# keurfonluu/stochopy

Hardware: AMD Instinct MI355X
Metric: objective-fn evals/sec (higher is better)
Workload: dtype f64

## Files before the change

include/stochopy_hip.h:

```cpp
#ifndef STOCHOPY_HIP_H
#define STOCHOPY_HIP_H

#include <stdint.h>

#ifdef __cplusplus
extern "C" {
#endif

#define SX_ABI_VERSION 1

enum {
    SX_FUN_ACKLEY = 0,
    SX_FUN_GRIEWANK = 1,
    SX_FUN_QUARTIC = 2,
    SX_FUN_RASTRIGIN = 3,
    SX_FUN_ROSENBROCK = 4,
    SX_FUN_SPHERE = 5,
    SX_FUN_STYBLINSKI_TANG = 6,
    SX_FUN_COUNT = 7
};

enum { SX_DE_RAND1BIN = 0, SX_DE_RAND2BIN = 1, SX_DE_BEST1BIN = 2, SX_DE_BEST2BIN = 3 };

enum {
// ... 4 lines not shown
#define SX_STATUS_NONE 100

int sx_abi_version(void);
const char *sx_last_error(void);
int sx_device_count(void);
int sx_struct_size(int which);

int sx_sum_plan(int64_t m, int32_t *out, int cap);
int64_t sx_fun_terms(int fun_id, int n);

int64_t sx_num_partials(int64_t P, int n);
int sx_rows_per_workgroup(int n);
int sx_wide_from(void);
int64_t sx_de_num_partials(int64_t P, int n, int wide_from);
int sx_eval(int fun_id, const double *X, int64_t P, int n, int64_t ldx, const double *xm, const double *xstd,
            double *f, double *part_f, int64_t *part_i, void *stream);

int sx_philox_lhs(double *X, int64_t rows, int n, int64_t ld, int64_t row0, int64_t P, const double *lower,
                  const double *upper, uint32_t key0, uint32_t key1, void *stream);

int sx_argmin(const double *f, int64_t P, double *ws_f, int64_t *ws_i, int64_t ws_len, int64_t *out_idx,
              double *out_val, void *stream);

typedef struct sx_state {
    int64_t it;
    int64_t gbidx;
    double gfit;
    double dx;
    int32_t status;
    int32_t done;
    int64_t reserved[3];
} sx_state;

typedef struct sx_de_args {
    double *buf0, *buf1;
    double *fit;
    double *candfit;
    double *gbest;
    const double *lower;
    const double *upper;
    sx_state *state;
    double *part_f;
    int64_t *part_i;
    const double *r1;
    const int32_t *donors;
    const int32_t *irand;
    const double *resample;
    int64_t P;
    int64_t ld;
    int64_t row0;
    int32_t n;
    int32_t fun_id;
    int32_t strategy;
    int32_t constraints;
    int32_t rng;
    int32_t maxiter;
    int32_t wide_from;
    int32_t pad;
    double F, CR, xtol, ftol;
    uint32_t key0, key1;
} sx_de_args;

int sx_de_generation(const sx_de_args *a, int finalize, void *stream);

int sx_select_finalize(const double *part_f, const int64_t *part_i, int64_t npart, const double *rows0,
                       const double *rows1, int64_t ld, int n, double *gbest, sx_state *state, int maxiter,
                       double xtol, double ftol, void *stream);

int sx_shard_best(const double *part_f, const int64_t *part_i, int64_t npart, const double *rows0,
                  const double *rows1, int64_t ld, int n, const sx_state *state, int64_t row0, double *record,
                  void *stream);
int sx_gather_finalize(const double *records, int world, int n, double *gbest, sx_state *state, int maxiter,
                       double xtol, double ftol, void *stream);
int sx_de_shard_generation(const struct sx_de_args *a, double *record, void *stream);

typedef struct sx_graph sx_graph;
int sx_de_graph_create(const sx_de_args *a, int ngen, sx_graph **out);
int sx_de_chain_launch(const sx_de_args *a, int parity, int finalize_only, void *stream);
int sx_de_chain_graph_create(const sx_de_args *a, int ngen, int start_parity, sx_graph **out);
int sx_graph_launch(sx_graph *g, void *stream);
int sx_graph_destroy(sx_graph *g);

#define SX_MAX_PEERS 8
#define SX_IPC_HANDLE_BYTES 64
typedef struct sx_xchg_args {
    uint64_t *peer[SX_MAX_PEERS];
    int32_t world, rank;
    int64_t timeout_ticks;
    int32_t *error;
    uint64_t *relay;
    const double *pop0[SX_MAX_PEERS];
    const double *pop1[SX_MAX_PEERS];
// ... 204 lines not shown
```

stochopy_amd/_lib.py:

```python
import ctypes as C
import os

_HERE = os.path.dirname(os.path.abspath(__file__))
LIB_PATH = os.path.join(_HERE, "lib", "libstochopy_hip.so")

SX_STATUS_NONE = 100
NARROW_DIM, WIDE_DIM = 4096, 262144


def wide_from():
    return int(lib().sx_wide_from())
SX_RNG_HOST, SX_RNG_PHILOX = 0, 1

FUN_IDS = {
    "ackley": 0,
    "griewank": 1,
    "quartic": 2,
    "rastrigin": 3,
    "rosenbrock": 4,
    "sphere": 5,
    "styblinski_tang": 6,
}
DE_STRATEGIES = {"rand1bin": 0, "rand2bin": 1, "best1bin": 2, "best2bin": 3}
DE_DONORS = {"rand1bin": 3, "rand2bin": 5, "best1bin": 2, "best2bin": 4}

vp = C.c_void_p
i64 = C.c_int64
i32 = C.c_int32
f64 = C.c_double


class SxState(C.Structure):
    _fields_ = [("it", i64), ("gbidx", i64), ("gfit", f64), ("dx", f64), ("status", i32), ("done", i32),
                ("reserved", i64 * 3)]


class SxDeArgs(C.Structure):
    _fields_ = [
        ("buf0", vp), ("buf1", vp), ("fit", vp), ("candfit", vp), ("gbest", vp), ("lower", vp),
        ("upper", vp), ("state", vp), ("part_f", vp), ("part_i", vp), ("r1", vp), ("donors", vp),
        ("irand", vp), ("resample", vp),
        ("P", i64), ("ld", i64), ("row0", i64),
        ("n", i32), ("fun_id", i32), ("strategy", i32), ("constraints", i32), ("rng", i32), ("maxiter", i32),
        ("wide_from", i32), ("pad", i32),
        ("F", f64), ("CR", f64), ("xtol", f64), ("ftol", f64),
        ("key0", C.c_uint32), ("key1", C.c_uint32),
    ]


class SxPsoArgs(C.Structure):
    _fields_ = [
        ("X", vp), ("V", vp), ("pbest", vp), ("pbestfit", vp), ("candfit", vp), ("gbest", vp), ("lower", vp),
        ("upper", vp), ("state", vp), ("part_f", vp), ("part_i", vp), ("r1", vp), ("r2", vp), ("pending_restart", vp),
        ("P", i64), ("ld", i64), ("row0", i64),
        ("n", i32), ("fun_id", i32), ("constraints", i32), ("rng", i32), ("maxiter", i32), ("pad", i32),
        ("w", f64), ("c1", f64), ("c2", f64), ("xtol", f64), ("ftol", f64),
        ("key0", C.c_uint32), ("key1", C.c_uint32),
    ]


SX_MAX_PEERS = 8
SX_IPC_HANDLE_BYTES = 64


class SxXchgArgs(C.Structure):
    _fields_ = [("peer", vp * SX_MAX_PEERS), ("world", i32), ("rank", i32), ("timeout_ticks", i64), ("error", vp),
                ("relay", vp), ("pop0", vp * SX_MAX_PEERS), ("pop1", vp * SX_MAX_PEERS), ("global_rows", i64),
                ("shard_rows", i64)]


class SxCmaState(C.Structure):
    _fields_ = [("it", i64), ("nfev", i64), ("best_row", i64), ("fbest", f64), ("sigma", f64), ("sigma_next", f64),
                ("tmp_coef", f64), ("psnorm", f64), ("status", i32), ("done", i32), ("stop_it", i64),
                ("reserved", f64 * 6)]


class SxVdArgs(C.Structure):
    _fields_ = [
# ... 159 lines not shown
```

stochopy_amd/csrc/sx_async.hip:

```cpp
#ifndef SX_ASYNC_PART
#define SX_ASYNC_PART 0
#endif
#define SX_FUSED_TAIL_BY_LANE 0
#include "sx_device.hpp"
#include "sx_host.hpp"
#include "sx_rowops.hpp"

namespace sx {
int make_plan_arg(int fun_id, int n, PlanArg *out);
}
using namespace sx;

namespace {

#ifndef SX_SWEEP_WAVES
#define SX_SWEEP_WAVES 16
#endif
constexpr int kSweepWaves = SX_SWEEP_WAVES;
__host__ __device__ constexpr int sweep_waves(int fun_id) {
    return (fun_id == SX_FUN_ACKLEY || fun_id == SX_FUN_GRIEWANK) ? (kSweepWaves + 1) / 2 : kSweepWaves;
}
constexpr int kSweepSlots = 64;

struct SweepGeometry {
// ... 335 lines not shown
template <int RNG, int LPR, int NFIX = 0>
pso_async_t pick_pso(int fun_id) {
    switch (fun_id) {
        case SX_FUN_ACKLEY: return pso_async_kernel<SX_FUN_ACKLEY, RNG, LPR, NFIX>;
        case SX_FUN_RASTRIGIN: return pso_async_kernel<SX_FUN_RASTRIGIN, RNG, LPR, NFIX>;
        case SX_FUN_ROSENBROCK: return pso_async_kernel<SX_FUN_ROSENBROCK, RNG, LPR, NFIX>;
        case SX_FUN_SPHERE: return pso_async_kernel<SX_FUN_SPHERE, RNG, LPR, NFIX>;
        case SX_FUN_GRIEWANK: return pso_async_kernel<SX_FUN_GRIEWANK, RNG, LPR, 0>;
        case SX_FUN_QUARTIC: return pso_async_kernel<SX_FUN_QUARTIC, RNG, LPR, 0>;
        case SX_FUN_STYBLINSKI_TANG: return pso_async_kernel<SX_FUN_STYBLINSKI_TANG, RNG, LPR, 0>;
    }
    return nullptr;
}

template <typename K>
int launch_sweep(K kern, const SweepGeometry &g, hipStream_t s, const void *args_struct) {
    (void)args_struct;
    SX_HIP(hipFuncSetAttribute(reinterpret_cast<const void *>(kern), hipFuncAttributeMaxDynamicSharedMemorySize,
                               (int)g.lds));
    return 0;
}

}

#if SX_ASYNC_PART == 0
extern "C" int sx_de_async_generation(const sx_de_args *a, void *stream) {
    SX_REQUIRE(a != nullptr, "sx_de_async: null args");
    SX_REQUIRE(a->buf0 && a->fit && a->gbest && a->state, "sx_de_async: null device pointer");
    SX_REQUIRE(a->P >= 2 && a->P < (int64_t)1 << 31 && a->n >= 1 && a->n <= kMaxDim && a->ld >= a->n, "sx_de_async: bad shape");
    SX_REQUIRE(a->fun_id >= 0 && a->fun_id < SX_FUN_COUNT, "sx_de_async: unknown objective");
    SX_REQUIRE(a->strategy >= 0 && a->strategy <= SX_DE_BEST2BIN, "sx_de_async: unknown strategy");
    SX_REQUIRE(a->P - 1 >= donors_of(a->strategy), "sx_de_async: population too small for the strategy");
    SX_REQUIRE(a->rng == SX_RNG_HOST || a->rng == SX_RNG_PHILOX, "sx_de_async: unknown rng mode");
    SX_REQUIRE(a->rng != SX_RNG_HOST || (a->r1 && a->donors && a->irand), "sx_de_async: host draws missing");
    SX_REQUIRE(a->constraints == 0 || (a->lower && a->upper && (a->rng != SX_RNG_HOST || a->resample)),
               "sx_de_async: bounds / resample draws missing");
    PlanArg plan;
    if (make_plan_arg(a->fun_id, a->n, &plan)) return -1;
    de_async_t kern = nullptr;
    if (a->rng == SX_RNG_PHILOX) {
        SX_DISPATCH_LPR(a->n, kern = a->n == 4 * LPR ? (pick_de<SX_RNG_PHILOX, LPR, 4 * LPR>(a->fun_id))
                                                      : (pick_de<SX_RNG_PHILOX, LPR>(a->fun_id)))
    } else {
        SX_DISPATCH_LPR(a->n, kern = (pick_de<SX_RNG_HOST, LPR>(a->fun_id)))
    }
    const SweepGeometry g = sweep_geometry(a->n, 0, a->fun_id);
    if (int rc = launch_sweep(kern, g, (hipStream_t)stream, a)) return rc;
    hipLaunchKernelGGL(kern, dim3(1), dim3(g.waves * kWave), g.lds, (hipStream_t)stream, *a, plan);
    SX_LAUNCH_CHECK();
    return 0;
}

#else
extern "C" int sx_pso_async_generation(const sx_pso_args *a, void *stream) {
    SX_REQUIRE(a != nullptr, "sx_pso_async: null args");
    SX_REQUIRE(a->X && a->V && a->pbest && a->pbestfit && a->gbest && a->state, "sx_pso_async: null device pointer");
    SX_REQUIRE(a->P >= 2 && a->n >= 1 && a->n <= kMaxDim && a->ld >= a->n, "sx_pso_async: bad shape");
    SX_REQUIRE(a->fun_id >= 0 && a->fun_id < SX_FUN_COUNT, "sx_pso_async: unknown objective");
    SX_REQUIRE(a->rng == SX_RNG_HOST || a->rng == SX_RNG_PHILOX, "sx_pso_async: unknown rng mode");
    SX_REQUIRE(a->rng != SX_RNG_HOST || (a->r1 && a->r2), "sx_pso_async: host draws missing");
    SX_REQUIRE(a->constraints == 0 || (a->lower && a->upper), "sx_pso_async: bounds missing");
    PlanArg plan;
    if (make_plan_arg(a->fun_id, a->n, &plan)) return -1;
    pso_async_t kern = nullptr;
    if (a->rng == SX_RNG_PHILOX) {
        SX_DISPATCH_LPR(a->n, kern = a->n == 4 * LPR ? (pick_pso<SX_RNG_PHILOX, LPR, 4 * LPR>(a->fun_id))
// ... 12 lines not shown
```

stochopy_amd/csrc/sx_de.hip:

```cpp
#define SX_DE_XM 0
#include "sx_de_kernel.hpp"
#include "sx_wide.hpp"

namespace sx {
void *de_chain_kernel(int fun_id, int n, int64_t P, int strategy, int constraints);
void *de_p2p_kernel(int fun_id, int n, int64_t P, int strategy, int constraints);
}

namespace {

int check_args(const sx_de_args *a) {
    SX_REQUIRE(a != nullptr, "sx_de: null args");
    SX_REQUIRE(a->buf0 && a->buf1 && a->fit && a->state && a->part_f && a->part_i, "sx_de: null device pointer");
    SX_REQUIRE(a->P >= 2 && a->P < (int64_t)1 << 31 && a->n >= 1 && a->ld >= a->n, "sx_de: bad shape");
    SX_REQUIRE(a->fun_id >= 0 && a->fun_id < SX_FUN_COUNT, "sx_de: unknown objective");
    SX_REQUIRE(a->strategy >= 0 && a->strategy <= 3, "sx_de: unknown strategy");
    SX_REQUIRE(a->P - 1 >= donors_of(a->strategy), "sx_de: popsize too small for the strategy");
    SX_REQUIRE(a->rng == SX_RNG_HOST || a->rng == SX_RNG_PHILOX, "sx_de: unknown rng mode");
    if (a->rng == SX_RNG_HOST) {
        SX_REQUIRE(a->r1 && a->donors && a->irand, "sx_de: host draws missing");
        SX_REQUIRE(a->constraints == 0 || a->resample, "sx_de: resample block missing");
    }
    SX_REQUIRE(a->constraints == 0 || (a->lower && a->upper), "sx_de: bounds missing");
    return 0;
}

de_kernel_t kernel_for(const sx_de_args *a) {
    return a->rng == SX_RNG_PHILOX ? pick_kernel<SX_RNG_PHILOX, 0>(a->fun_id, a->n, a->P, a->strategy, a->constraints)
                                   : pick_kernel<SX_RNG_HOST, 0>(a->fun_id, a->n, a->P, a->strategy, a->constraints);
}

Geometry geometry(const sx_de_args *a) {
    Geometry g = row_geometry(a->P, a->n, de_wide_from(a));
    if (!is_wide(a->n, de_wide_from(a))) g.lds = (size_t)rows_per_block(a->n) * gen_row_stride(a->n) * sizeof(double);
    return g;
}

}

extern "C" int sx_de_generation(const sx_de_args *a, int finalize, void *stream) {
    if (int rc = check_args(a)) return rc;
    hipStream_t s = (hipStream_t)stream;
    const Geometry g = geometry(a);
    if (is_wide(a->n, de_wide_from(a))) {
        if (int rc = wide_de_launch(a, s)) return rc;
    } else {
        PlanArg plan;
        if (make_plan_arg(a->fun_id, a->n, &plan)) return -1;
        hipLaunchKernelGGL(kernel_for(a), dim3(g.blocks), dim3(g.threads), g.lds, s, (const sx_state *)nullptr,
                           (const double *)nullptr, (const int64_t *)nullptr, (int64_t)g.blocks, *a, plan, 0, 0,
                           sx_xchg_args{});
        SX_LAUNCH_CHECK();
    }
    if (finalize) {
        SX_REQUIRE(a->gbest != nullptr, "sx_de_generation: the separate finalize kernel needs the gbest buffer");
        return sx_select_finalize(a->part_f, a->part_i, g.blocks, a->buf0, a->buf1, a->ld, a->n, a->gbest, a->state,
                                  a->maxiter, a->xtol, a->ftol, stream);
    }
    return 0;
}

extern "C" int sx_de_graph_create(const sx_de_args *a, int ngen, sx_graph **out) {
    if (int rc = check_args(a)) return rc;
    SX_REQUIRE(out != nullptr && ngen >= 1 && a->gbest != nullptr, "sx_de_graph_create: bad arguments");
    SX_REQUIRE(a->rng == SX_RNG_PHILOX, "sx_de_graph_create: graphs need in-kernel (Philox) draws");
    PlanArg plan = {};
    const bool wide = is_wide(a->n, de_wide_from(a));
    if (!wide && make_plan_arg(a->fun_id, a->n, &plan)) return -1;
    const Geometry g = geometry(a);
    sx_graph *gr = new sx_graph();
    SX_HIP(hipGraphCreate(&gr->graph, 0));
    sx_de_args args = *a;
    int zero = 0;
    int64_t npart = g.blocks;
    sx_xchg_args nox = {};
    const void *none = nullptr;
    void *kargs[] = {&none, &none, &none, &npart, &args, &plan, &zero, &zero, &nox};
    hipGraphNode_t prev = nullptr;
    for (int i = 0; i < ngen; ++i) {
        if (wide) {
            if (int rc = wide_de_add_node(gr->graph, &prev, a)) return rc;
        } else {
            hipKernelNodeParams kp = {};
            kp.func = (void *)kernel_for(a);
            kp.gridDim = dim3(g.blocks);
            kp.blockDim = dim3(g.threads);
            kp.sharedMemBytes = (unsigned)g.lds;
            kp.kernelParams = kargs;
            kp.extra = nullptr;
            hipGraphNode_t node;
            SX_HIP(hipGraphAddKernelNode(&node, gr->graph, prev ? &prev : nullptr, prev ? 1 : 0, &kp));
            prev = node;
        }
        if (int rc = add_finalize_node(gr->graph, &prev, a->part_f, a->part_i, g.blocks, a->buf0, a->buf1, a->ld, a->n,
                                       a->gbest, a->state, a->maxiter, a->xtol, a->ftol))
            return rc;
    }
    SX_HIP(hipGraphInstantiate(&gr->exec, gr->graph, nullptr, nullptr, 0));
    *out = gr;
    return 0;
}

extern "C" int sx_de_shard_generation(const sx_de_args *a, double *record, void *stream) {
    SX_REQUIRE(record != nullptr, "sx_de_shard_generation: null record");
    if (int rc = sx_de_generation(a, 0, stream)) return rc;
    return sx_shard_best(a->part_f, a->part_i, (int64_t)geometry(a).blocks, a->buf0, a->buf1, a->ld, a->n, a->state,
                         a->row0, record, stream);
}

static int check_chain(const sx_de_args *a, bool peer_exchange) {
    if (int rc = check_args(a)) return rc;
    SX_REQUIRE(a->rng == SX_RNG_PHILOX, "sx_de_chain: needs in-kernel (Philox) draws");
    SX_REQUIRE(!is_wide(a->n, de_wide_from(a)), "sx_de_chain: rows served by the one-workgroup-per-row kernels (n > wide_from) take the two-kernel path (sx_de_generation)");
    SX_REQUIRE(peer_exchange || geometry(a).blocks <= 512,
               "sx_de_chain: more than 512 workgroup records (use the two-kernel path)");
    return 0;
}

static int chain_launch(const sx_de_args *a, const sx_xchg_args *x, int parity, int finalize_only, void *stream) {
    if (int rc = check_chain(a, x != nullptr)) return rc;
    SX_REQUIRE(parity == 0 || parity == 1, "sx_de_chain_launch: parity must be 0 or 1");
    PlanArg plan;
    if (make_plan_arg(a->fun_id, a->n, &plan)) return -1;
    const Geometry g = geometry(a);
    de_kernel_t kern = (de_kernel_t)(x ? de_p2p_kernel(a->fun_id, a->n, a->P, a->strategy, a->constraints)
                                       : de_chain_kernel(a->fun_id, a->n, a->P, a->strategy, a->constraints));
    const unsigned blocks = finalize_only ? 1u : g.blocks + (x ? 1u : 0u);
    hipLaunchKernelGGL(kern, dim3(blocks), dim3(g.threads), g.lds, (hipStream_t)stream,
                       (const sx_state *)(a->state + parity), (const double *)(a->part_f + (int64_t)parity * g.blocks),
                       (const int64_t *)(a->part_i + (int64_t)parity * g.blocks), (int64_t)g.blocks, *a, plan, parity,
                       finalize_only ? 1 : 0, x ? *x : sx_xchg_args{});
    SX_LAUNCH_CHECK();
    return 0;
}

static int chain_graph_create(const sx_de_args *a, const sx_xchg_args *x, int ngen, int start_parity, sx_graph **out) {
    if (int rc = check_chain(a, x != nullptr)) return rc;
    SX_REQUIRE(out != nullptr && ngen >= 1 && (start_parity == 0 || start_parity == 1),
               "sx_de_chain_graph_create: bad arguments");
    PlanArg plan;
    if (make_plan_arg(a->fun_id, a->n, &plan)) return -1;
    const Geometry g = geometry(a);
    sx_graph *gr = new sx_graph();
    SX_HIP(hipGraphCreate(&gr->graph, 0));
    sx_de_args args = *a;
    sx_xchg_args xa = x ? *x : sx_xchg_args{};
    int mode = 0;
    int64_t npart = g.blocks;
    hipGraphNode_t prev = nullptr;
    for (int i = 0; i < ngen; ++i) {
        int parity = (start_parity + i) & 1;
        const sx_state *sin_pre = a->state + parity;
        const double *pf_pre = a->part_f + (int64_t)parity * npart;
        const int64_t *pi_pre = a->part_i + (int64_t)parity * npart;
        void *kargs[] = {&sin_pre, &pf_pre, &pi_pre, &npart, &args, &plan, &parity, &mode, &xa};
        hipKernelNodeParams kp = {};
        kp.func = x ? de_p2p_kernel(a->fun_id, a->n, a->P, a->strategy, a->constraints)
                    : de_chain_kernel(a->fun_id, a->n, a->P, a->strategy, a->constraints);
        kp.gridDim = dim3(g.blocks + (x ? 1u : 0u));
        kp.blockDim = dim3(g.threads);
        kp.sharedMemBytes = (unsigned)g.lds;
        kp.kernelParams = kargs;
        kp.extra = nullptr;
        hipGraphNode_t node;
        SX_HIP(hipGraphAddKernelNode(&node, gr->graph, prev ? &prev : nullptr, prev ? 1 : 0, &kp));
        prev = node;
    }
    SX_HIP(hipGraphInstantiate(&gr->exec, gr->graph, nullptr, nullptr, 0));
    *out = gr;
    return 0;
}

extern "C" int sx_de_chain_launch(const sx_de_args *a, int parity, int finalize_only, void *stream) {
    return chain_launch(a, nullptr, parity, finalize_only, stream);
}
extern "C" int sx_de_chain_graph_create(const sx_de_args *a, int ngen, int start_parity, sx_graph **out) {
    return chain_graph_create(a, nullptr, ngen, start_parity, out);
}

extern "C" int sx_de_p2p_launch(const sx_de_args *a, const sx_xchg_args *x, int parity, int finalize_only,
                                void *stream) {
    if (int rc = check_xchg_args(x)) return rc;
    return chain_launch(a, x, parity, finalize_only, stream);
}
extern "C" int sx_de_p2p_graph_create(const sx_de_args *a, const sx_xchg_args *x, int ngen, int start_parity,
                                      sx_graph **out) {
    if (int rc = check_xchg_args(x)) return rc;
    return chain_graph_create(a, x, ngen, start_parity, out);
// ... 17 lines not shown
```

stochopy_amd/csrc/sx_de_kernel.hpp:

```cpp
#pragma once
#ifndef SX_DE_XM
#error "define SX_DE_XM (0, 1 or 2) before including sx_de_kernel.hpp"
#endif
#include <type_traits>
#include <vector>

#include "sx_device.hpp"
#include "sx_host.hpp"
#include "sx_rowops.hpp"
#include "sx_xchg.hpp"

namespace sx {
int make_plan_arg(int fun_id, int n, PlanArg *out);
int add_finalize_node(hipGraph_t graph, hipGraphNode_t *prev, const double *part_f, const int64_t *part_i,
                      int64_t npart, const double *rows0, const double *rows1, int64_t ld, int n, double *gbest,
                      sx_state *state, int maxiter, double xtol, double ftol);
int check_xchg_args(const sx_xchg_args *x);
}
using namespace sx;

#if defined(SX_TRACE) && SX_DE_XM == 1
__device__ unsigned long long sx_trace_buf[1024 * 16];
#define SX_TP(k)                                                                              \
    do {                                                                                      \
// ... 117 lines not shown
        int status = SX_STATUS_NONE;
        if (it >= 2) {
            if (gf <= a.ftol)
                status = 1;
            else if (it >= a.maxiter)
                status = -1;
        }
        sx_state *so = a.state + (mode == 1 ? 2 : 1 - chain_p);
        so->it = it;
        so->gbidx = gi;
        so->gfit = gf;
        so->dx = 0.0;
        so->status = status;
        so->done = status != SX_STATUS_NONE;
        so->reserved[0] = prev_winner;
        so->reserved[1] = winner;
    }
}

constexpr int kStep = 4;

#ifndef SX_DE_NFIX_WAVES
#define SX_DE_NFIX_WAVES 1
#endif
#ifndef SX_DE_WAVE_ROWS_WAVES
#define SX_DE_WAVE_ROWS_WAVES 1
#endif
template <int FUN, int RNG, int XM, int LPR, bool FULL, int NFIX = 0, int STRAT = -1, bool ONEB = false>
__global__ __launch_bounds__(kMaxWavesPerBlock *kWave, (NFIX != 0 && XM <= 1) ? SX_DE_NFIX_WAVES
                                                       : (NFIX == 0 && XM == 0 && STRAT >= 0 && LPR == kWave) ? SX_DE_WAVE_ROWS_WAVES
                                                                                                                 : 1) void de_generation_kernel(const sx_state *const sin_pre,
                                                                                 const double *const pf_pre,
                                                                                 const int64_t *const pi_pre,
                                                                                 const int64_t npart,
                                                                                 const sx_de_args a,
                                                                                 const PlanArg plan,
                                                                                 const int chain_p, const int mode,
                                                                                 const sx_xchg_args x) {
    constexpr bool CHAIN = XM >= 1;
    constexpr bool P2P = XM == 2;
    extern __shared__ __attribute__((aligned(16))) double lds[];
    __shared__ double sf[kMaxRowsPerBlock];
    __shared__ int64_t si[kMaxRowsPerBlock];
    __shared__ double s_gf;
    __shared__ int64_t s_gi;
    __shared__ int s_winner;
    SX_TP(0);
    const int n = NFIX ? NFIX : a.n;
    const int64_t P = a.P, ld = a.ld;
    const RowIds<LPR> id(P, P2P ? 1 : 0);
    const int l = id.l;
    const int64_t rowc = id.rowc;
    double *U = lds + id.slot * gen_row_stride(n);

    const sx_state *sin = (CHAIN && !P2P) ? sin_pre : CHAIN ? a.state + chain_p : a.state;
    constexpr int kRecPerLane = 8;
    double pfv[kRecPerLane];
    using rec_t = typename std::conditional<LPR == kWave, int32_t, int64_t>::type;
    constexpr rec_t kNoRec = LPR == kWave ? (rec_t)INT32_MAX : (rec_t)INT64_MAX;
    rec_t piv[kRecPerLane];
#ifndef SX_CHAIN_REC_WAVE0
#define SX_CHAIN_REC_WAVE0 1
#endif
    if (CHAIN && !P2P && (!SX_CHAIN_REC_WAVE0 || id.wave == 0)) {
        const double *pf = pf_pre;
        const int64_t *pi = pi_pre;
        const int per = (int)((npart + kWave - 1) / kWave);
        const int64_t k0 = (int64_t)id.lane * per;
#pragma unroll
        for (int u = 0; u < kRecPerLane; ++u) {
            const bool in = u < per && k0 + u < npart;
            pfv[u] = in ? pf[k0 + u] : __builtin_huge_val();
            piv[u] = in ? (rec_t)pi[k0 + u] : kNoRec;
        }
    }
    if (P2P && blockIdx.x == 0) {
        p2p_service(a, x, chain_p, mode, npart, sin, LPR == kWave);
        return;
    }
    if (sin->done) {
        if (CHAIN && mode == 1 && threadIdx.x == 0) a.state[2] = *sin;
        return;
    }
    const int64_t it = CHAIN ? sin->it + 1 : sin->it;
    SX_TP(6);

    const uint32_t gen = (uint32_t)(it + 1);
    const double *__restrict__ cur = (it & 1) ? a.buf1 : a.buf0;
    double *__restrict__ nxt = (it & 1) ? a.buf0 : a.buf1;
    const double fold = a.fit[rowc];
    const double *__restrict__ xi = cur + rowc * ld;
    const uint32_t grow = (uint32_t)(a.row0 + rowc);
    const int strategy = STRAT >= 0 ? STRAT : a.strategy;
    const int k = donors_of(strategy);
    const bool repair = STRAT >= 0 ? false : a.constraints != 0;
    const bool use_best = strategy == SX_DE_BEST1BIN || strategy == SX_DE_BEST2BIN;

    int64_t d[kMaxDonors];
    int irand;
    const bool gdon = P2P && x.global_rows > 0;
    if (RNG == SX_RNG_PHILOX) {
        philox_donors(gdon ? x.global_rows : P, k, gdon ? a.row0 + rowc : rowc, grow, gen, a.key0, a.key1, n, d, irand);
    } else {
#pragma unroll
        for (int t = 0; t < kMaxDonors; ++t) d[t] = t < k ? (int64_t)a.donors[(int64_t)t * P + rowc] : 0;
        irand = a.irand[rowc];
    }
    SX_TP(1);
// ... 229 lines not shown
            for (int t = 0; t < kStep; ++t) {
                const int e = (q0 + t) * LPR + l;
                g[t] = (use_best && (FULL || e < n)) ? gb[e] : 0.0;
            }
        }
#pragma unroll
        for (int t = 0; t < kStep; ++t) {
            const int e = (q0 + t) * LPR + l;
            if (FULL || e < n) {
                const double v = de_mutant(strategy, g[t], bd[0][t], bd[1][t], bd[2][t], bd[3][t], bd[4][t], F);
                double cand = (e == irand || br[t] <= CR) ? v : bx[t];
                if (repair && (cand < a.lower[e] || cand > a.upper[e])) cand = brs[t];
                U[e] = cand;
                if (kRegRow) keep[t] = cand;
            }
        }
    };
    if constexpr (LPR < kWave) {
        trial_batch(0, B0);
    } else {
        trial_batch(0, B0);
        if constexpr (!ONEB) {
            for (int q0 = kStep; q0 < nq; q0 += kStep) {
                load_batch(q0, B0);
                trial_batch(q0, B0);
            }
        }
    }

    SX_TP(2);
    const double fc = row_objective<FUN, LPR, FULL, NFIX, SX_LONG_STATIC, ONEB>(U, n, plan, l);
    SX_TP(3);
    const bool better = fc < fold;
    if (FULL || id.active) {
        double *__restrict__ xo = nxt + id.row * ld;
        if constexpr (kRegRow) {
#pragma unroll
            for (int t = 0; t < kStep; ++t)
                if (NFIX != 0 || l + t * LPR < n) st_stream(xo + l + t * LPR, better ? keep[t] : B0.x[t]);
        } else {
            const double *__restrict__ src = better ? U : xi;
            for (int e0 = l; e0 < n; e0 += kStep * LPR) {
                double v[kStep];
#pragma unroll
                for (int t = 0; t < kStep; ++t) v[t] = (FULL || e0 + t * LPR < n) ? src[e0 + t * LPR] : 0.0;
#pragma unroll
                for (int t = 0; t < kStep; ++t)
                    if (FULL || e0 + t * LPR < n) xo[e0 + t * LPR] = v[t];
            }
        }
        if (l == 0) {
            if (better) a.fit[id.row] = fc;
            if (a.candfit != nullptr) a.candfit[id.row] = fc;
        }
    }
    SX_TP(4);
    block_partial<LPR>(better ? fc : fold, id, sf, si, part_f_out, part_i_out);
    SX_TP(5);
}

typedef void (*de_kernel_t)(const sx_state *, const double *, const int64_t *, const int64_t, const sx_de_args,
                            const PlanArg, const int, const int, const sx_xchg_args);

template <int RNG, int XM, int LPR, bool FULL, int NFIX = 0, int STRAT = -1, bool ONEB = false>
de_kernel_t pick_kernel_lpr(int fun_id) {
    constexpr bool SPECIAL = STRAT != -1 || ONEB || NFIX != 0;
    switch (fun_id) {
        case SX_FUN_ACKLEY: return de_generation_kernel<SX_FUN_ACKLEY, RNG, XM, LPR, FULL, NFIX, STRAT, ONEB>;
        case SX_FUN_RASTRIGIN: return de_generation_kernel<SX_FUN_RASTRIGIN, RNG, XM, LPR, FULL, NFIX, STRAT, ONEB>;
        case SX_FUN_ROSENBROCK: return de_generation_kernel<SX_FUN_ROSENBROCK, RNG, XM, LPR, FULL, NFIX, STRAT, ONEB>;
        case SX_FUN_SPHERE: return de_generation_kernel<SX_FUN_SPHERE, RNG, XM, LPR, FULL, NFIX, STRAT, ONEB>;
    }
    if constexpr (!SPECIAL) {
        switch (fun_id) {
            case SX_FUN_GRIEWANK: return de_generation_kernel<SX_FUN_GRIEWANK, RNG, XM, LPR, FULL, NFIX, STRAT, ONEB>;
            case SX_FUN_QUARTIC: return de_generation_kernel<SX_FUN_QUARTIC, RNG, XM, LPR, FULL, NFIX, STRAT, ONEB>;
            case SX_FUN_STYBLINSKI_TANG: return de_generation_kernel<SX_FUN_STYBLINSKI_TANG, RNG, XM, LPR, FULL, NFIX, STRAT, ONEB>;
        }
    }
    return nullptr;
}

template <int RNG, int XM, int LPR, bool FULL, int NFIX>
de_kernel_t pick_kernel_fixed(int fun_id, int strategy, int constraints) {
    if constexpr (XM == 2 && LPR != 32) {
        return pick_kernel_lpr<RNG, XM, LPR, FULL, NFIX>(fun_id);
    } else {
        if (constraints != 0 || !hot_objective(fun_id)) return pick_kernel_lpr<RNG, XM, LPR, FULL, NFIX>(fun_id);
        switch (strategy) {
            case SX_DE_RAND1BIN: return pick_kernel_lpr<RNG, XM, LPR, FULL, NFIX, NFIX ? SX_DE_RAND1BIN : -1>(fun_id);
            case SX_DE_BEST1BIN: return pick_kernel_lpr<RNG, XM, LPR, FULL, NFIX, NFIX ? SX_DE_BEST1BIN : -1>(fun_id);
        }
        return pick_kernel_lpr<RNG, XM, LPR, FULL, NFIX>(fun_id);
    }
}
// ... 38 lines not shown
```

stochopy_amd/csrc/sx_rowops.hpp:

```cpp
#pragma once
#include "sx_device.hpp"

namespace sx {

template <int LPR>
struct RowIds {
    static constexpr int RPW = kWave / LPR;
    int wave, lane;
    int l;
    int slot;
    int block;
    int64_t row, rowc;
    bool active;
    __device__ __forceinline__ explicit RowIds(int64_t P, int first_block = 0) {
        wave = (int)(threadIdx.x >> 6);
        lane = (int)(threadIdx.x & 63);
        l = lane & (LPR - 1);
        slot = wave * RPW + lane / LPR;
        const int rows_in_block = (int)(blockDim.x >> 6) * RPW;
        block = (int)blockIdx.x - first_block;
        row = (int64_t)block * rows_in_block + slot;
        active = row < P;
        rowc = active ? row : P - 1;
    }
// ... 321 lines not shown
            const int e = e0 + t * LPR;
            x[t] = (FULL || e < m) ? U[e] : 0.0;
            xn[t] = (O::NEXT && (FULL || e < m)) ? U[e + 1] : 0.0;
        }
#pragma unroll
        for (int t = 0; t < 4; ++t) {
            const int e = e0 + t * LPR;
            if (e < m) {
                double a, b;
                O::term(x[t], xn[t], e, a, b);
                A[e] = a;
                if (O::TWO) B[e] = b;
            }
        }
    }
    lds_wave_fence();
    double sa, sb;
    if constexpr (NFIX != 0 && NFIX <= 256) {
        if constexpr (!O::NEXT)
            row_reduce_fixed<O::TWO, O::BMUL, LPR, NFIX>(A, B, l, sa, sb);
        else
            row_reduce_static<O::TWO, O::BMUL, NFIX - 1>(A, B, l, sa, sb);
        return O::finish(sa, sb, n);
    }
    if (plan.nleaf > 1)
        row_reduce_leaves<O::TWO, O::BMUL, LPR>(A, B, B + n, B + n + 24, leaf_cap(n), plan, l, sa, sb);
    else
        row_reduce2<O::TWO, O::BMUL>(A, B, B + n, plan, l, sa, sb);
    return O::finish(sa, sb, n);
}

template <int LPR>
__device__ __forceinline__ void block_partial(double val, const RowIds<LPR> &id, double *sf, int64_t *si,
                                              double *__restrict__ part_f, int64_t *__restrict__ part_i) {
    if (id.l == 0) {
        sf[id.slot] = id.active ? val : __builtin_huge_val();
        si[id.slot] = id.active ? id.row : INT64_MAX;
    }
    __syncthreads();
    if (threadIdx.x < kWave) {
        const int rows_in_block = (int)(blockDim.x >> 6) * RowIds<LPR>::RPW;
        const int k = (int)threadIdx.x;
        double bf = k < rows_in_block ? sf[k] : __builtin_huge_val();
        int64_t bi = k < rows_in_block ? si[k] : INT64_MAX;
        wave_argmin_ordered(bf, bi);
        if (k == 0) {
            part_f[id.block] = bf;
            part_i[id.block] = bi;
        }
    }
}

constexpr int kMaxDonors = 5;

__host__ __device__ inline int donors_of(int strategy) {
    return strategy == SX_DE_RAND1BIN ? 3 : strategy == SX_DE_RAND2BIN ? 5 : strategy == SX_DE_BEST1BIN ? 2 : 4;
}

__device__ __forceinline__ void philox_donors(int64_t P, int k, int64_t i, uint32_t grow, uint32_t gen, uint32_t k0,
                                              uint32_t k1, int n, int64_t (&d)[kMaxDonors], int &irand) {
    const U4 a = philox4x32_10(0u, grow, gen, kPurposeDeDonor, k0, k1);
    U4 b = {0u, 0u, 0u, 0u};
    if (k > 3) b = philox4x32_10(1u, grow, gen, kPurposeDeDonor, k0, k1);
    const uint32_t w[5] = {a.y, a.z, a.w, b.x, b.y};
    uint32_t excl[kMaxDonors + 1];
    excl[0] = (uint32_t)i;
    const uint32_t Pm1 = (uint32_t)(P - 1);
#pragma unroll
    for (int t = 0; t < kMaxDonors; ++t) {
        if (t < k) {
            uint32_t v = __umulhi(w[t], Pm1 - (uint32_t)t);
#pragma unroll
            for (int s = 0; s <= t; ++s) v += (v >= excl[s]) ? 1u : 0u;
            d[t] = (int64_t)v;
            uint32_t carry = v;
#pragma unroll
            for (int s = 0; s <= t; ++s) {
                if (carry < excl[s]) {
                    const uint32_t tmp = excl[s];
                    excl[s] = carry;
                    carry = tmp;
// ... 32 lines not shown
```

stochopy_amd/csrc/sx_unfused.hip:

```cpp
#include "sx_device.hpp"
#include "sx_host.hpp"
#include "sx_rowops.hpp"

using namespace sx;

namespace {

constexpr int kStep = 4;

template <int RNG, int LPR>
__global__ __launch_bounds__(kMaxWavesPerBlock *kWave) void de_propose_kernel(const sx_de_args a,
                                                                              double *__restrict__ cand) {
    const sx_state *st = a.state;
    if (st->done) return;
    const int n = a.n;
    const int64_t P = a.P, ld = a.ld;
    const RowIds<LPR> id(P);
    if (!id.active) return;
    const int l = id.l;
    const int64_t row = id.row, it = st->it;
    const uint32_t gen = (uint32_t)(it + 1), grow = (uint32_t)(a.row0 + row);
    const double *__restrict__ cur = (it & 1) ? a.buf1 : a.buf0;
    const double *__restrict__ xi = cur + row * ld;
    const int strategy = a.strategy, k = donors_of(strategy);
// ... 138 lines not shown
template <int LPR>
__global__ __launch_bounds__(kMaxWavesPerBlock *kWave) void rows_select_kernel(
    const double *__restrict__ cand, int64_t ldc, const double *__restrict__ f, const double *xin, double *xout,
    int64_t ldx, double *__restrict__ xfun, double *__restrict__ candfit, int64_t P, int n, const sx_state *st,
    double *__restrict__ part_f, int64_t *__restrict__ part_i) {
    __shared__ double sf[kMaxRowsPerBlock];
    __shared__ int64_t si[kMaxRowsPerBlock];
    if (st->done) return;
    const RowIds<LPR> id(P);
    const double fc = f[id.rowc], fold = xfun[id.rowc];
    const bool better = fc < fold;
    if (id.active) {
        const double *src = better ? cand + id.row * ldc : xin + id.row * ldx;
        double *dst = xout + id.row * ldx;
        if (better || xin != xout)
            for (int e = id.l; e < n; e += LPR) dst[e] = src[e];
        if (id.l == 0) {
            if (better) xfun[id.row] = fc;
            if (candfit != nullptr) candfit[id.row] = fc;
        }
    }
    block_partial<LPR>(better ? fc : fold, id, sf, si, part_f, part_i);
}

}

extern "C" int sx_de_propose(const sx_de_args *a, double *cand, void *stream) {
    SX_REQUIRE(a != nullptr && cand != nullptr, "sx_de_propose: null pointer");
    SX_REQUIRE(a->buf0 && a->buf1 && a->state, "sx_de_propose: null device pointer");
    SX_REQUIRE(a->P >= 2 && a->P < (int64_t)1 << 31 && a->n >= 1 && a->ld >= a->n, "sx_de_propose: bad shape");
    SX_REQUIRE(a->strategy >= 0 && a->strategy <= SX_DE_BEST2BIN, "sx_de_propose: unknown strategy");
    SX_REQUIRE(a->P - 1 >= donors_of(a->strategy), "sx_de_propose: population too small for the strategy");
    SX_REQUIRE(a->rng == SX_RNG_HOST || a->rng == SX_RNG_PHILOX, "sx_de_propose: unknown rng mode");
    SX_REQUIRE(a->rng != SX_RNG_HOST || (a->r1 && a->donors && a->irand), "sx_de_propose: host draws missing");
    SX_REQUIRE(a->constraints == 0 || (a->lower && a->upper && (a->rng != SX_RNG_HOST || a->resample)),
               "sx_de_propose: bounds / resample draws missing");
    const Geometry g = row_geometry(a->P, a->n, run_wide_from(a->wide_from));
    if (a->rng == SX_RNG_PHILOX) {
        SX_DISPATCH_LPR(a->n, hipLaunchKernelGGL((de_propose_kernel<SX_RNG_PHILOX, LPR>), dim3(g.blocks), dim3(g.threads), 0,
                                                 (hipStream_t)stream, *a, cand))
    } else {
        SX_DISPATCH_LPR(a->n, hipLaunchKernelGGL((de_propose_kernel<SX_RNG_HOST, LPR>), dim3(g.blocks), dim3(g.threads), 0,
                                                 (hipStream_t)stream, *a, cand))
    }
    SX_LAUNCH_CHECK();
    return 0;
}

extern "C" int sx_pso_move(const sx_pso_args *a, void *stream) {
    SX_REQUIRE(a != nullptr, "sx_pso_move: null args");
    SX_REQUIRE(a->X && a->V && a->pbest && a->gbest && a->state, "sx_pso_move: null device pointer");
    SX_REQUIRE(a->P >= 2 && a->n >= 1 && a->ld >= a->n, "sx_pso_move: bad shape");
    SX_REQUIRE(a->rng == SX_RNG_HOST || a->rng == SX_RNG_PHILOX, "sx_pso_move: unknown rng mode");
    SX_REQUIRE(a->rng != SX_RNG_HOST || (a->r1 && a->r2), "sx_pso_move: host draws missing");
    SX_REQUIRE(a->constraints == 0 || (a->lower && a->upper), "sx_pso_move: bounds missing");
    const Geometry g = row_geometry(a->P, a->n, kWideFrom);
    const size_t lds = a->n > kWideFrom ? 0 : (size_t)rows_per_block(a->n) * a->n * sizeof(double);
    if (a->rng == SX_RNG_PHILOX) {
        SX_DISPATCH_LPR(a->n, hipLaunchKernelGGL((pso_move_kernel<SX_RNG_PHILOX, LPR>), dim3(g.blocks), dim3(g.threads), lds,
                                                 (hipStream_t)stream, *a, lds != 0 ? 1 : 0))
    } else {
        SX_DISPATCH_LPR(a->n, hipLaunchKernelGGL((pso_move_kernel<SX_RNG_HOST, LPR>), dim3(g.blocks), dim3(g.threads), lds,
                                                 (hipStream_t)stream, *a, lds != 0 ? 1 : 0))
    }
    SX_LAUNCH_CHECK();
    return 0;
// ... 14 lines not shown
```

stochopy_amd/optimize/_de.py:

```python
import ctypes as C
import os
import warnings

import numpy as np

from .. import _device, _lib, _rng
from . import _common
from ._helpers import register
from ._population import _PopulationRun

__all__ = ["minimize"]


def minimize(
    fun,
    bounds,
    x0=None,
    args=(),
    maxiter=100,
    popsize=10,
    mutation=0.5,
    recombination=0.9,
    strategy="best1bin",
    seed=None,
# ... 74 lines not shown
            if smallest < 2:
                raise ValueError(f"popsize {self.Ptotal} over {self.world.size} ranks leaves {smallest} row(s) on the last GPU: "
                                 "a shard needs at least 2")
            if (self.Ptotal if self.global_donors else smallest) - 1 < self.k:
                raise ValueError(f"strategy {strategy} draws {self.k} donors: too few rows "
                                 f"({'population' if self.global_donors else 'smallest shard'} of "
                                 f"{self.Ptotal if self.global_donors else smallest})")
        needs_narrow = (self.world is not None and self.external is None
                        and (donors == "global" or (exchange or os.environ.get("SX_EXCHANGE")) == "p2p"))
        self.wide_from = _lib.NARROW_DIM if needs_narrow else 0
        self.wide = self.n > (self.wide_from or _lib.wide_from())
        self.npart = int(_lib.lib().sx_de_num_partials(self.P, self.n, self.wide_from))
        self.chain = (rng == "philox" and self.world is None and callback is None and not return_all
                      and self.npart <= 512 and not immediate and self.external is None and not self.wide)
        self.ctx = _device.Context()
        if self.world is not None:
            exchange = exchange or os.environ.get("SX_EXCHANGE") or "auto"
            if exchange not in ("auto", "p2p", "rccl"):
                raise ValueError('exchange must be "auto", "p2p" or "rccl"')
            if self.external is not None and (exchange == "p2p" or self.global_donors):
                raise ValueError("a caller-supplied objective runs between kernels: the peer exchange lives "
                                 'inside the fused generation kernel (use exchange="rccl", donors="shard")')
            if self.wide and (exchange == "p2p" or self.global_donors):
                raise ValueError(f"rows of {self.n} elements (> {_lib.NARROW_DIM}) exchange the global best with one "
                                 'all-gather per generation (exchange="rccl", donors="shard")')
            if self.external is not None or self.wide:
                exchange = "rccl"
        self.px, self.exchange, self.exchange_note = self._negotiate_exchange(exchange)
        if self.px is not None:
            self.chain = True
        if self.global_donors and self.px is None:
            raise RuntimeError('donors="global" needs the peer exchange (exchange="p2p"/"auto"): '
                               f'{self.exchange_note or "it was switched off"}')
        self._tail_seen = {}
        self._shard_calls = None
        self._rccl_tail_seen = {}
        if autorun:
            self._autorun()

    def close(self):
        if self.global_donors and self.px is not None:
            self.bufs = None
        super().close()

    def read_state(self):
        st = super().read_state()
        self.it_enq = int(st.it)
        return st

    def _chain_launch(self, parity, finalize_only):
        ctx = self.ctx
        if self.px is not None:
            _lib.check(ctx.L.sx_de_p2p_launch(C.byref(self.args), C.byref(self.px.args), parity, finalize_only,
                                              ctx.stream_ptr), "sx_de_p2p_launch")
        else:
            _lib.check(ctx.L.sx_de_chain_launch(C.byref(self.args), parity, finalize_only, ctx.stream_ptr),
                       "sx_de_chain_launch")

    def _create_chain_graph(self, par, size):
        g = C.c_void_p()
        if self.px is not None:
            _lib.check(self.ctx.L.sx_de_p2p_graph_create(C.byref(self.args), C.byref(self.px.args), size, par, C.byref(g)),
                       "sx_de_p2p_graph_create")
        else:
            _lib.check(self.ctx.L.sx_de_chain_graph_create(C.byref(self.args), size, par, C.byref(g)),
                       "sx_de_chain_graph_create")
# ... 133 lines not shown
            from ..parallel import best_of_records

            self.record = ctx.empty((n + 2,))
            self.records = ctx.empty((self.world.size, n + 2))
            self.record[0] = gfit0
            self.record[1] = float(self.row0 + g)
            self.record[2:].copy_(self.gbest)
            self.world.all_gather_records(self.record, self.records)
            wbest, gfit0, g = best_of_records(self.records.cpu().numpy())
            self.gbest.copy_(self.records[wbest, 2:])
        st = _lib.SxState(it=1, gbidx=g, gfit=gfit0, dx=0.0, status=_lib.SX_STATUS_NONE, done=0)
        if self.chain:
            s0 = _lib.SxState(it=0, gbidx=g, gfit=gfit0, dx=0.0, status=_lib.SX_STATUS_NONE, done=0)
            raw = np.frombuffer(bytes(s0) + bytes(st) + bytes(st), dtype=np.int64).copy()
            self.state = ctx.upload_async(raw)
            if quiet_start:
                self.part_f, self.part_i = rec_f, rec_i
            else:
                pf = np.full((2, npart), np.inf)
                pi = np.full((2, npart), np.iinfo(np.int64).max, dtype=np.int64)
                pf[0, 0], pi[0, 0] = gfit0, g
                self.part_f = ctx.upload(pf)
                self.part_i = ctx.upload(pi)
        else:
            self.state = ctx.upload(np.frombuffer(bytes(st), dtype=np.int64).copy())
        key0, key1 = _rng.philox_key(self.seed) if self.rng == "philox" else (0, 0)
        a = _lib.SxDeArgs()
        a.buf0, a.buf1 = self.bufs[0].data_ptr(), self.bufs[1].data_ptr()
        if self.immediate:
            a.buf0 = a.buf1
        a.fit, a.candfit = self.fit.data_ptr(), self.candfit.data_ptr()
        a.lower, a.upper, a.state = self.d_lower.data_ptr(), self.d_upper.data_ptr(), self.state.data_ptr()
        a.part_f, a.part_i = self.part_f.data_ptr(), self.part_i.data_ptr()
        a.gbest = None if self.chain else self.gbest.data_ptr()
        a.P, a.ld, a.row0, a.n = P, n, self.row0, n
        a.wide_from = self.wide_from
        a.fun_id, a.strategy = (self.fun_id if self.external is None else 0), _lib.DE_STRATEGIES[self.strategy]
        if self.external is not None:
            self.cand = ctx.empty((P, n))
            self.cand_f = ctx.empty((P,))
        self.it_enq = 1
        a.constraints = 1 if self.constraints == "Random" else 0
        a.rng = _lib.SX_RNG_PHILOX if self.rng == "philox" else _lib.SX_RNG_HOST
        a.maxiter = self.maxiter
        a.F, a.CR, a.xtol, a.ftol = self.F, self.CR, self.xtol, self.ftol
        a.key0, a.key1 = key0, key1
        self.args = a
        if self.rng == "numpy-legacy":
            self.h_r1 = t.empty((P, n), dtype=t.float64).pin_memory()
            self.h_don = t.empty((self.k, P), dtype=t.int32).pin_memory()
            self.h_irand = t.empty((P,), dtype=t.int32).pin_memory()
            self.d_r1 = ctx.empty((P, n))
            self.d_don = ctx.empty((self.k, P), dtype=t.int32)
            self.d_irand = ctx.empty((P,), dtype=t.int32)
            a.r1, a.donors, a.irand = self.d_r1.data_ptr(), self.d_don.data_ptr(), self.d_irand.data_ptr()
            if a.constraints:
                self.h_rs = t.empty((P, n), dtype=t.float64).pin_memory()
                self.d_rs = ctx.empty((P, n))
                a.resample = self.d_rs.data_ptr()
        self.st = st
        if self.world is not None and (self.return_all or self.callback is not None):
            self.Xfull = ctx.empty((self.Ptotal, n))
            self.candfull = ctx.empty((self.Ptotal,))
            if self.px is not None:
                st = self.read_state()
                self.gbest.copy_(ctx.upload(self._best_row(st)))
# ... 154 lines not shown
```

Measured before the change: 602.8 million.

## Skip rewriting unchanged DE rows using per-block winner bitmasks

Adds a per-workgroup 16-bit mask, double-buffered by parity, that records which rows took a trial vector in the previous generation. In the single-GPU chained kernel, a row is written to the next buffer only if it improved now or changed last generation. Otherwise the ping-pong buffer already holds the same data from two generations back. This is meant to cut global memory write traffic, at the cost of a ballot, extra LDS, a small mask read and write per block, and a repacked kernel argument list.

```diff
diff --git a/include/stochopy_hip.h b/include/stochopy_hip.h
--- a/include/stochopy_hip.h
+++ b/include/stochopy_hip.h
@@ -60,6 +60,7 @@
     int64_t reserved[3];
 } sx_state;
 
+#define SX_DE_ROWBITS_SET 512
 typedef struct sx_de_args {
     double *buf0, *buf1;
     double *fit;
@@ -86,6 +87,7 @@
     int32_t wide_from;
     int32_t pad;
     double F, CR, xtol, ftol;
+    uint16_t *rowbits;
     uint32_t key0, key1;
 } sx_de_args;
 
diff --git a/stochopy_amd/_lib.py b/stochopy_amd/_lib.py
--- a/stochopy_amd/_lib.py
+++ b/stochopy_amd/_lib.py
@@ -21,6 +21,7 @@
     "sphere": 5,
     "styblinski_tang": 6,
 }
+SX_DE_ROWBITS_SET = 512
 DE_STRATEGIES = {"rand1bin": 0, "rand2bin": 1, "best1bin": 2, "best2bin": 3}
 DE_DONORS = {"rand1bin": 3, "rand2bin": 5, "best1bin": 2, "best2bin": 4}
 
@@ -43,7 +44,7 @@
         ("P", i64), ("ld", i64), ("row0", i64),
         ("n", i32), ("fun_id", i32), ("strategy", i32), ("constraints", i32), ("rng", i32), ("maxiter", i32),
         ("wide_from", i32), ("pad", i32),
-        ("F", f64), ("CR", f64), ("xtol", f64), ("ftol", f64),
+        ("F", f64), ("CR", f64), ("xtol", f64), ("ftol", f64), ("rowbits", vp),
         ("key0", C.c_uint32), ("key1", C.c_uint32),
     ]
 
diff --git a/stochopy_amd/csrc/sx_async.hip b/stochopy_amd/csrc/sx_async.hip
--- a/stochopy_amd/csrc/sx_async.hip
+++ b/stochopy_amd/csrc/sx_async.hip
@@ -391,6 +391,7 @@
     SX_REQUIRE(a->strategy >= 0 && a->strategy <= SX_DE_BEST2BIN, "sx_de_async: unknown strategy");
     SX_REQUIRE(a->P - 1 >= donors_of(a->strategy), "sx_de_async: population too small for the strategy");
     SX_REQUIRE(a->rng == SX_RNG_HOST || a->rng == SX_RNG_PHILOX, "sx_de_async: unknown rng mode");
+    SX_REQUIRE(a->rowbits == nullptr, "sx_de_async: row bits (rowbits) serve the single-GPU chained kernel only");
     SX_REQUIRE(a->rng != SX_RNG_HOST || (a->r1 && a->donors && a->irand), "sx_de_async: host draws missing");
     SX_REQUIRE(a->constraints == 0 || (a->lower && a->upper && (a->rng != SX_RNG_HOST || a->resample)),
                "sx_de_async: bounds / resample draws missing");
diff --git a/stochopy_amd/csrc/sx_de.hip b/stochopy_amd/csrc/sx_de.hip
--- a/stochopy_amd/csrc/sx_de.hip
+++ b/stochopy_amd/csrc/sx_de.hip
@@ -25,6 +25,12 @@
     return 0;
 }
 
+int check_plain(const sx_de_args *a) {
+    if (int rc = check_args(a)) return rc;
+    SX_REQUIRE(a->rowbits == nullptr, "sx_de: row bits (rowbits) serve the single-GPU chained kernel only");
+    return 0;
+}
+
 de_kernel_t kernel_for(const sx_de_args *a) {
     return a->rng == SX_RNG_PHILOX ? pick_kernel<SX_RNG_PHILOX, 0>(a->fun_id, a->n, a->P, a->strategy, a->constraints)
                                    : pick_kernel<SX_RNG_HOST, 0>(a->fun_id, a->n, a->P, a->strategy, a->constraints);
@@ -39,7 +45,7 @@
 }
 
 extern "C" int sx_de_generation(const sx_de_args *a, int finalize, void *stream) {
-    if (int rc = check_args(a)) return rc;
+    if (int rc = check_plain(a)) return rc;
     hipStream_t s = (hipStream_t)stream;
     const Geometry g = geometry(a);
     if (is_wide(a->n, de_wide_from(a))) {
@@ -48,7 +54,7 @@
         PlanArg plan;
         if (make_plan_arg(a->fun_id, a->n, &plan)) return -1;
         hipLaunchKernelGGL(kernel_for(a), dim3(g.blocks), dim3(g.threads), g.lds, s, (const sx_state *)nullptr,
-                           (const double *)nullptr, (const int64_t *)nullptr, (int64_t)g.blocks, *a, plan, 0, 0,
+                           (const double *)nullptr, (const int64_t *)nullptr, (int32_t)g.blocks, (int32_t)0, *a, plan,
                            sx_xchg_args{});
         SX_LAUNCH_CHECK();
     }
@@ -61,7 +67,7 @@
 }
 
 extern "C" int sx_de_graph_create(const sx_de_args *a, int ngen, sx_graph **out) {
-    if (int rc = check_args(a)) return rc;
+    if (int rc = check_plain(a)) return rc;
     SX_REQUIRE(out != nullptr && ngen >= 1 && a->gbest != nullptr, "sx_de_graph_create: bad arguments");
     SX_REQUIRE(a->rng == SX_RNG_PHILOX, "sx_de_graph_create: graphs need in-kernel (Philox) draws");
     PlanArg plan = {};
@@ -71,11 +77,11 @@
     sx_graph *gr = new sx_graph();
     SX_HIP(hipGraphCreate(&gr->graph, 0));
     sx_de_args args = *a;
-    int zero = 0;
-    int64_t npart = g.blocks;
+    int32_t zero = 0;
+    int32_t npart = (int32_t)g.blocks;
     sx_xchg_args nox = {};
     const void *none = nullptr;
-    void *kargs[] = {&none, &none, &none, &npart, &args, &plan, &zero, &zero, &nox};
+    void *kargs[] = {&none, &none, &none, &npart, &zero, &args, &plan, &nox};
     hipGraphNode_t prev = nullptr;
     for (int i = 0; i < ngen; ++i) {
         if (wide) {
@@ -109,10 +115,10 @@
 }
 
 static int check_chain(const sx_de_args *a, bool peer_exchange) {
-    if (int rc = check_args(a)) return rc;
+    if (int rc = peer_exchange ? check_plain(a) : check_args(a)) return rc;
     SX_REQUIRE(a->rng == SX_RNG_PHILOX, "sx_de_chain: needs in-kernel (Philox) draws");
     SX_REQUIRE(!is_wide(a->n, de_wide_from(a)), "sx_de_chain: rows served by the one-workgroup-per-row kernels (n > wide_from) take the two-kernel path (sx_de_generation)");
-    SX_REQUIRE(peer_exchange || geometry(a).blocks <= 512,
+    SX_REQUIRE(peer_exchange || geometry(a).blocks <= SX_DE_ROWBITS_SET,
                "sx_de_chain: more than 512 workgroup records (use the two-kernel path)");
     return 0;
 }
@@ -128,8 +134,8 @@
     const unsigned blocks = finalize_only ? 1u : g.blocks + (x ? 1u : 0u);
     hipLaunchKernelGGL(kern, dim3(blocks), dim3(g.threads), g.lds, (hipStream_t)stream,
                        (const sx_state *)(a->state + parity), (const double *)(a->part_f + (int64_t)parity * g.blocks),
-                       (const int64_t *)(a->part_i + (int64_t)parity * g.blocks), (int64_t)g.blocks, *a, plan, parity,
-                       finalize_only ? 1 : 0, x ? *x : sx_xchg_args{});
+                       (const int64_t *)(a->part_i + (int64_t)parity * g.blocks), (int32_t)g.blocks,
+                       (int32_t)(parity | (finalize_only ? 2 : 0)), *a, plan, x ? *x : sx_xchg_args{});
     SX_LAUNCH_CHECK();
     return 0;
 }
@@ -145,15 +151,14 @@
     SX_HIP(hipGraphCreate(&gr->graph, 0));
     sx_de_args args = *a;
     sx_xchg_args xa = x ? *x : sx_xchg_args{};
-    int mode = 0;
-    int64_t npart = g.blocks;
+    int32_t npart = (int32_t)g.blocks;
     hipGraphNode_t prev = nullptr;
     for (int i = 0; i < ngen; ++i) {
-        int parity = (start_parity + i) & 1;
+        int32_t parity = (start_parity + i) & 1;
         const sx_state *sin_pre = a->state + parity;
         const double *pf_pre = a->part_f + (int64_t)parity * npart;
         const int64_t *pi_pre = a->part_i + (int64_t)parity * npart;
-        void *kargs[] = {&sin_pre, &pf_pre, &pi_pre, &npart, &args, &plan, &parity, &mode, &xa};
+        void *kargs[] = {&sin_pre, &pf_pre, &pi_pre, &npart, &parity, &args, &plan, &xa};
         hipKernelNodeParams kp = {};
         kp.func = x ? de_p2p_kernel(a->fun_id, a->n, a->P, a->strategy, a->constraints)
                     : de_chain_kernel(a->fun_id, a->n, a->P, a->strategy, a->constraints);
diff --git a/stochopy_amd/csrc/sx_de_kernel.hpp b/stochopy_amd/csrc/sx_de_kernel.hpp
--- a/stochopy_amd/csrc/sx_de_kernel.hpp
+++ b/stochopy_amd/csrc/sx_de_kernel.hpp
@@ -173,16 +173,19 @@
                                                                                                                  : 1) void de_generation_kernel(const sx_state *const sin_pre,
                                                                                  const double *const pf_pre,
                                                                                  const int64_t *const pi_pre,
-                                                                                 const int64_t npart,
+                                                                                 const int32_t npart32,
+                                                                                 const int32_t parity_mode,
                                                                                  const sx_de_args a,
                                                                                  const PlanArg plan,
-                                                                                 const int chain_p, const int mode,
                                                                                  const sx_xchg_args x) {
+    const int64_t npart = npart32;
+    const int chain_p = parity_mode & 1, mode = parity_mode >> 1;
     constexpr bool CHAIN = XM >= 1;
     constexpr bool P2P = XM == 2;
     extern __shared__ __attribute__((aligned(16))) double lds[];
     __shared__ double sf[kMaxRowsPerBlock];
     __shared__ int64_t si[kMaxRowsPerBlock];
+    __shared__ int sbit[kMaxRowsPerBlock];
     __shared__ double s_gf;
     __shared__ int64_t s_gi;
     __shared__ int s_winner;
@@ -215,6 +218,8 @@
             piv[u] = in ? (rec_t)pi[k0 + u] : kNoRec;
         }
     }
+    const bool rbits = XM == 1 && a.rowbits != nullptr;
+    const uint32_t won_word = rbits ? a.rowbits[(int64_t)chain_p * SX_DE_ROWBITS_SET + id.block] : 0u;
     if (P2P && blockIdx.x == 0) {
         p2p_service(a, x, chain_p, mode, npart, sin, LPR == kWave);
         return;
@@ -510,7 +515,9 @@
     const double fc = row_objective<FUN, LPR, FULL, NFIX, SX_LONG_STATIC, ONEB>(U, n, plan, l);
     SX_TP(3);
     const bool better = fc < fold;
-    if (FULL || id.active) {
+    const int rows_in_block = (int)(blockDim.x >> 6) * RowIds<LPR>::RPW;
+    const bool won_before = !rbits || ((won_word >> (rowc - (int64_t)id.block * rows_in_block)) & 1) != 0;
+    if ((FULL || id.active) && (better || won_before)) {
         double *__restrict__ xo = nxt + id.row * ld;
         if constexpr (kRegRow) {
 #pragma unroll
@@ -527,18 +534,19 @@
                     if (FULL || e0 + t * LPR < n) xo[e0 + t * LPR] = v[t];
             }
         }
-        if (l == 0) {
-            if (better) a.fit[id.row] = fc;
-            if (a.candfit != nullptr) a.candfit[id.row] = fc;
-        }
+    }
+    if ((FULL || id.active) && l == 0) {
+        if (better) a.fit[id.row] = fc;
+        if (a.candfit != nullptr) a.candfit[id.row] = fc;
     }
     SX_TP(4);
-    block_partial<LPR>(better ? fc : fold, id, sf, si, part_f_out, part_i_out);
+    block_partial<LPR>(better ? fc : fold, id, sf, si, part_f_out, part_i_out,
+                       rbits ? a.rowbits + (int64_t)(1 - chain_p) * SX_DE_ROWBITS_SET : nullptr, sbit, better);
     SX_TP(5);
 }
 
-typedef void (*de_kernel_t)(const sx_state *, const double *, const int64_t *, const int64_t, const sx_de_args,
-                            const PlanArg, const int, const int, const sx_xchg_args);
+typedef void (*de_kernel_t)(const sx_state *, const double *, const int64_t *, const int32_t, const int32_t, const sx_de_args,
+                            const PlanArg, const sx_xchg_args);
 
 template <int RNG, int XM, int LPR, bool FULL, int NFIX = 0, int STRAT = -1, bool ONEB = false>
 de_kernel_t pick_kernel_lpr(int fun_id) {
diff --git a/stochopy_amd/csrc/sx_rowops.hpp b/stochopy_amd/csrc/sx_rowops.hpp
--- a/stochopy_amd/csrc/sx_rowops.hpp
+++ b/stochopy_amd/csrc/sx_rowops.hpp
@@ -377,10 +377,13 @@
 
 template <int LPR>
 __device__ __forceinline__ void block_partial(double val, const RowIds<LPR> &id, double *sf, int64_t *si,
-                                              double *__restrict__ part_f, int64_t *__restrict__ part_i) {
+                                              double *__restrict__ part_f, int64_t *__restrict__ part_i,
+                                              uint16_t *__restrict__ bits_out = nullptr, int *sbit = nullptr,
+                                              bool bit = false) {
     if (id.l == 0) {
         sf[id.slot] = id.active ? val : __builtin_huge_val();
         si[id.slot] = id.active ? id.row : INT64_MAX;
+        if (bits_out != nullptr) sbit[id.slot] = id.active && bit;
     }
     __syncthreads();
     if (threadIdx.x < kWave) {
@@ -389,9 +392,11 @@
         double bf = k < rows_in_block ? sf[k] : __builtin_huge_val();
         int64_t bi = k < rows_in_block ? si[k] : INT64_MAX;
         wave_argmin_ordered(bf, bi);
+        const unsigned long long bits = bits_out != nullptr ? __ballot(k < rows_in_block && sbit[k] != 0) : 0ull;
         if (k == 0) {
             part_f[id.block] = bf;
             part_i[id.block] = bi;
+            if (bits_out != nullptr) bits_out[id.block] = (uint16_t)bits;
         }
     }
 }
diff --git a/stochopy_amd/csrc/sx_unfused.hip b/stochopy_amd/csrc/sx_unfused.hip
--- a/stochopy_amd/csrc/sx_unfused.hip
+++ b/stochopy_amd/csrc/sx_unfused.hip
@@ -194,6 +194,7 @@
     SX_REQUIRE(a->strategy >= 0 && a->strategy <= SX_DE_BEST2BIN, "sx_de_propose: unknown strategy");
     SX_REQUIRE(a->P - 1 >= donors_of(a->strategy), "sx_de_propose: population too small for the strategy");
     SX_REQUIRE(a->rng == SX_RNG_HOST || a->rng == SX_RNG_PHILOX, "sx_de_propose: unknown rng mode");
+    SX_REQUIRE(a->rowbits == nullptr, "sx_de_propose: row bits (rowbits) serve the single-GPU chained kernel only");
     SX_REQUIRE(a->rng != SX_RNG_HOST || (a->r1 && a->donors && a->irand), "sx_de_propose: host draws missing");
     SX_REQUIRE(a->constraints == 0 || (a->lower && a->upper && (a->rng != SX_RNG_HOST || a->resample)),
                "sx_de_propose: bounds / resample draws missing");
diff --git a/stochopy_amd/optimize/_de.py b/stochopy_amd/optimize/_de.py
--- a/stochopy_amd/optimize/_de.py
+++ b/stochopy_amd/optimize/_de.py
@@ -130,6 +130,7 @@
         if self.global_donors and self.px is None:
             raise RuntimeError('donors="global" needs the peer exchange (exchange="p2p"/"auto"): '
                                f'{self.exchange_note or "it was switched off"}')
+        self.rowbits_on = self.chain and self.px is None and os.environ.get("SX_DE_STORE_ALL") != "1"
         self._tail_seen = {}
         self._shard_calls = None
         self._rccl_tail_seen = {}
@@ -329,6 +330,9 @@
         a.fit, a.candfit = self.fit.data_ptr(), self.candfit.data_ptr()
         a.lower, a.upper, a.state = self.d_lower.data_ptr(), self.d_upper.data_ptr(), self.state.data_ptr()
         a.part_f, a.part_i = self.part_f.data_ptr(), self.part_i.data_ptr()
+        if self.rowbits_on:
+            self.rowbits = t.full((2, _lib.SX_DE_ROWBITS_SET), -1, dtype=t.int16, device=ctx.device)
+            a.rowbits = self.rowbits.data_ptr()
         a.gbest = None if self.chain else self.gbest.data_ptr()
         a.P, a.ld, a.row0, a.n = P, n, self.row0, n
         a.wide_from = self.wide_from
```

Result: slower. 574.3 million, median of 6 (-4.7%).
